# tobwei/APTAI

Measured on AMD Instinct MI355X. Metric: utterances/sec (10 s @ 16 kHz) train-step, higher is better.
Workload: dtype bf16

## Files before the change

### aptai_amd/csrc/attention.hip

```cpp
#include "common.h"

namespace {

#ifdef APTAI_STAMPS
__device__ unsigned long long g_attn_stamps[3 * 1024 * 8];
#define ATTN_STAMP(k, slot)                                                                                       \
    do {                                                                                                          \
        if (threadIdx.x == 0) {                                                                                   \
            const int bl = blockIdx.x + gridDim.x * (blockIdx.y + gridDim.y * blockIdx.z);                        \
            if (bl < 1024) g_attn_stamps[((k) * 1024 + bl) * 8 + (slot)] = wall_clock64();                         \
        }                                                                                                         \
    } while (0)
#else
#define ATTN_STAMP(k, slot) do {} while (0)
#endif

constexpr int HD = 64;
constexpr float LOG2E = 1.4426950408889634f;

struct AttnArgs {
    const bf16_t* qkv; long ld;
    const int* lens;
    bf16_t* ctx; long ldo;
    float* lse2;
// ... 144 lines not shown
    const long tile_stride = 64 * a.ld;
#pragma unroll
    for (int it = 0; it < 2; ++it) { kreg[it] = *(const u32x4*)(Kg + goff[it]); vreg[it] = *(const u32x4*)(Vg + goff[it]); }
    uint32_t hbase = 0;
    if (DROP) hbase = rng_hash((uint32_t)((b * a.heads + hd) * a.Tp + q), a.seed0, a.seed1) + (uint32_t)(2 * h) * ATTN_K1;
    const float c = a.c;
#pragma unroll
    for (int it = 0; it < 2; ++it) { *(u32x4*)(smem + soff[it]) = kreg[it]; *(u32x4*)(smem + 64 * 128 + soff[it]) = vreg[it]; }
    if (ntiles > 1) {
#pragma unroll
        for (int it = 0; it < 2; ++it) {
            kreg[it] = *(const u32x4*)(Kg + tile_stride + goff[it]);
            vreg[it] = *(const u32x4*)(Vg + tile_stride + goff[it]);
        }
    }
    __syncthreads();
    ATTN_STAMP(0, 1);

    auto tile = [&](auto first_flag, auto mask_flag, const int t) {
        constexpr bool FIRST = decltype(first_flag)::value, MASK = decltype(mask_flag)::value;
        const char* sK = smem + (t & 1) * FWD_BUF;
        const char* sV = sK + 64 * 128;
        const int kbase = t * 64;
        bf16x8 kfr[2][4];
#pragma unroll
        for (int ds = 0; ds < 4; ++ds) kfr[0][ds] = rd_row(sK, lo, 0, ds);
        if (t + 1 < ntiles) {
            char* nb = smem + ((t + 1) & 1) * FWD_BUF;
#pragma unroll
            for (int it = 0; it < 2; ++it) { *(u32x4*)(nb + soff[it]) = kreg[it]; *(u32x4*)(nb + 64 * 128 + soff[it]) = vreg[it]; }
            if (t + 2 < ntiles) {
                const bf16_t* kn = Kg + (long)(t + 2) * tile_stride;
                const bf16_t* vn = Vg + (long)(t + 2) * tile_stride;
#pragma unroll
                for (int it = 0; it < 2; ++it) { kreg[it] = *(const u32x4*)(kn + goff[it]); vreg[it] = *(const u32x4*)(vn + goff[it]); }
            }
        }
        f32x16 sT[2];
        sT[0] = __builtin_amdgcn_mfma_f32_32x32x16_bf16(kfr[0][0], qf[0], (f32x16)(0.f), 0, 0, 0);
#pragma unroll
        for (int ds = 1; ds < 4; ++ds) sT[0] = __builtin_amdgcn_mfma_f32_32x32x16_bf16(kfr[0][ds], qf[ds], sT[0], 0, 0, 0);
#pragma unroll
        for (int ds = 0; ds < 4; ++ds) kfr[1][ds] = rd_row(sK, lo, 1, ds);
        sT[1] = __builtin_amdgcn_mfma_f32_32x32x16_bf16(kfr[1][0], qf[0], (f32x16)(0.f), 0, 0, 0);
#pragma unroll
        for (int ds = 1; ds < 4; ++ds) sT[1] = __builtin_amdgcn_mfma_f32_32x32x16_bf16(kfr[1][ds], qf[ds], sT[1], 0, 0, 0);
        if (MASK) {
#pragma unroll
            for (int kt2 = 0; kt2 < 2; ++kt2)
#pragma unroll
                for (int r = 0; r < 16; ++r)
                    if (kbase + kt2 * 32 + acc_row(r, h) >= len) sT[kt2][r] = -INFINITY;
        }
        if (FIRST) {
            float mt = sT[0][0];
#pragma unroll
            for (int r = 1; r < 16; ++r) mt = fmaxf(mt, sT[0][r]);
#pragma unroll
            for (int r = 0; r < 16; ++r) mt = fmaxf(mt, sT[1][r]);
            mt = fmaxf(mt, __shfl_xor(mt, 32, 64));
            ref = fmaf(mt, c, REF_HEADROOM);
        }
        float psum = 0.f;
#pragma unroll
        for (int kt2 = 0; kt2 < 2; ++kt2) {
            bf16x8 vfr[2][2];
#pragma unroll
            for (int s = 0; s < 2; ++s)
#pragma unroll
                for (int dt = 0; dt < 2; ++dt) vfr[s][dt] = rd_tr(sV, lo, 2 * kt2 + s, dt);
            float x[16];
#pragma unroll
            for (int r = 0; r < 16; ++r) { x[r] = fast_exp2(fmaf(sT[kt2][r], c, -ref)); psum += x[r]; }
            if (DROP) {
#pragma unroll
                for (int r = 0; r < 16; r += 2) {
                    const uint32_t hsh = attn_mix(hbase + (uint32_t)(kbase / 2 + 16 * kt2 + acc_row(r, 0) / 2) * ATTN_K1);
                    x[r] = (hsh & 0xffffu) >= a.thr16 ? x[r] : 0.f;
                    x[r + 1] = (hsh >> 16) >= a.thr16 ? x[r + 1] : 0.f;
                }
            }
            const bf16x8 pf0 = pack8(&x[0]), pf1 = pack8(&x[8]);
#pragma unroll
            for (int dt = 0; dt < 2; ++dt) oT[dt] = __builtin_amdgcn_mfma_f32_32x32x16_bf16(vfr[0][dt], pf0, oT[dt], 0, 0, 0);
#pragma unroll
            for (int dt = 0; dt < 2; ++dt) oT[dt] = __builtin_amdgcn_mfma_f32_32x32x16_bf16(vfr[1][dt], pf1, oT[dt], 0, 0, 0);
        }
        psum += __shfl_xor(psum, 32, 64);
        l_run += psum;
        if (!FIRST && __builtin_amdgcn_ballot_w64(!(psum <= REF_SUM_LIMIT))) {
            if (!(psum <= REF_SUM_LIMIT)) {
                const float e = floorf(fast_log2(psum)) + REF_HEADROOM;
                const float sc = fast_exp2(-e);
                ref += e;
                l_run *= sc;
#pragma unroll
                for (int r = 0; r < 16; ++r) { oT[0][r] *= sc; oT[1][r] *= sc; }
            }
        }
        __syncthreads();
    };
    if (ntiles == 1) {
        tile(Flag<true>{}, Flag<true>{}, 0);
    } else {
        tile(Flag<true>{}, Flag<false>{}, 0);
        for (int t = 1; t + 1 < ntiles; ++t) tile(Flag<false>{}, Flag<false>{}, t);
        tile(Flag<false>{}, Flag<true>{}, ntiles - 1);
    }
    ATTN_STAMP(0, 2);
    const float l_tot = l_run;
    const float inv = __frcp_rn(l_tot) * a.dscale;
    if (a.lse2 && h == 0) a.lse2[((long)b * a.heads + hd) * a.Tp + q] = ref + fast_log2(l_tot);
    char* sw = smem + wave * (32 * OUT_PITCH);
    const int r31 = lane & 31;
#pragma unroll
    for (int dt = 0; dt < 2; ++dt)
#pragma unroll
        for (int g4 = 0; g4 < 4; ++g4) {
            oT[dt][4 * g4 + 0] *= inv; oT[dt][4 * g4 + 1] *= inv; oT[dt][4 * g4 + 2] *= inv; oT[dt][4 * g4 + 3] *= inv;
            const int d = dt * 32 + 8 * g4 + 4 * h;
            *(u32x2*)(sw + r31 * OUT_PITCH + d * 2) = (u32x2){pack2bf(oT[dt][4 * g4], oT[dt][4 * g4 + 1]),
                                                              pack2bf(oT[dt][4 * g4 + 2], oT[dt][4 * g4 + 3])};
        }
    __syncthreads();
    const long orow = (rowbase + q0) * a.ldo + hd * HD;
#pragma unroll
    for (int i = 0; i < 4; ++i) {
        const int idx = i * 64 + lane, r = idx >> 3, ch = idx & 7;
        *(u32x4*)(a.ctx + orow + (long)r * a.ldo + ch * 8) = *(const u32x4*)(sw + r * OUT_PITCH + ch * 16);
    }
    if (a.o32) {
#pragma unroll
        for (int dt = 0; dt < 2; ++dt) {
            __syncthreads();
#pragma unroll
            for (int g4 = 0; g4 < 4; ++g4)
                *(f32x4*)(sw + r31 * OUT_PITCH + (8 * g4 + 4 * h) * 4) =
                    (f32x4){oT[dt][4 * g4], oT[dt][4 * g4 + 1], oT[dt][4 * g4 + 2], oT[dt][4 * g4 + 3]};
            __syncthreads();
#pragma unroll
            for (int i = 0; i < 4; ++i) {
                const int idx = i * 64 + lane, r = idx >> 3, ch = idx & 7;
                *(f32x4*)(a.o32 + orow + (long)r * a.ldo + dt * 32 + ch * 4) = *(const f32x4*)(sw + r * OUT_PITCH + ch * 16);
            }
        }
    }
    ATTN_STAMP(0, 3);
#ifdef APTAI_STAMPS
    asm volatile("s_waitcnt vmcnt(0)" ::: "memory");
    ATTN_STAMP(0, 4);
#endif
}

template <bool PRE>
__global__ __launch_bounds__(256, PRE ? DKDV_BLOCKS : 2) void attn_bwd_dkdv_kernel(AttnArgs a) {
    __shared__ __attribute__((aligned(16))) char smem[STAGE_BYTES + 384 + DKDV_KV_BYTES];
    char* sQ = smem;
    char* sD = smem + 32 * 128;
    float* sL = (float*)(smem + STAGE_BYTES);
    char* sKall = smem + STAGE_BYTES + 384;
    char* sVall = sKall + 128 * 128;
    ATTN_STAMP(1, 0);
    if (a.thr16) apply_salt(a.salt, a.seed0, a.seed1);
    const int tid = threadIdx.x, lane = tid & 63, wave = tid >> 6, h = lane >> 5;
    int tile_x, hd, b;
    attn_block(a, tile_x, hd, b);
    const int kb0 = tile_x * 128;
    const int key0 = kb0 + wave * 32;
    int len = a.lens[b];
    len = len < 1 ? 1 : (len > a.Tp ? a.Tp : len);
    const long rowbase = (long)b * a.Tp;
    const int key = key0 + (lane & 31);
    bf16_t* dK0 = a.dqkv + (rowbase + kb0) * a.ld + a.H + hd * HD;
    bf16_t* dV0 = dK0 + a.H;
    if (kb0 >= len) {
        const u32x4 z = {0u, 0u, 0u, 0u};
#pragma unroll
        for (int it = 0; it < 4; ++it) {
            const int cid = it * 256 + tid, row = cid >> 3, ch = cid & 7;
            *(u32x4*)(dK0 + (long)row * a.ld + ch * 8) = z;
            *(u32x4*)(dV0 + (long)row * a.ld + ch * 8) = z;
        }
        return;
    }
    const LaneOffs lo = lane_offs(lane);
    const bf16_t* K0 = a.qkv + (rowbase + kb0) * a.ld + a.H + hd * HD;
    stage_rows128(sKall, K0, a.ld, tid);
    stage_rows128(sVall, K0 + a.H, a.ld, tid);
    f32x16 dKT[2], dVT[2];
    dKT[0] = dKT[1] = dVT[0] = dVT[1] = (f32x16)(0.f);

    const int nq = a.skip_pad_q ? ((len + 31) >> 5) : (a.Tp >> 5);
    const bf16_t* Qb = a.qkv + rowbase * a.ld + hd * HD;
    const bf16_t* Db = a.dctx + rowbase * a.ldo + hd * HD;
    const float* lse = a.lse2 + ((long)b * a.heads + hd) * a.Tp;
    const float* del = a.delta + ((long)b * a.heads + hd) * a.Tp;
    const int srow = tid >> 3, sch = tid & 7;
    const int soff = tile_off(srow, sch);
    const long gq = (long)srow * a.ld + sch * 8, gd = (long)srow * a.ldo + sch * 8;
    u32x4 qreg = *(const u32x4*)(Qb + gq), dreg = *(const u32x4*)(Db + gd);
    const float* stat = (tid < 8 ? lse : del) + (tid & 7) * 4;
    f32x4 sreg = (f32x4)(0.f);
    if (tid < 16) sreg = *(const f32x4*)stat;
    const bool key_ok = key < len;
    const bool wave_boundary = key0 + 32 > len;
    const uint32_t hshift = (key & 1) ? 16u : 0u;
    const float c = a.c;
    const uint32_t pairk = (uint32_t)(key >> 1) * ATTN_K1;
    const uint32_t rowid0 = (uint32_t)((b * a.heads + hd) * a.Tp) + (uint32_t)(tid & 31);
    uint32_t hreg = 0;
    if (a.thr16 && tid >= 32 && tid < 64) hreg = rng_hash(rowid0, a.seed0, a.seed1);
    ATTN_STAMP(1, 1);
    for (int t = 0; t < nq; ++t) {
        __syncthreads();
        *(u32x4*)(sQ + soff) = qreg;
        *(u32x4*)(sD + soff) = dreg;
        if (tid < 16) *(f32x4*)(sL + tid * 4) = PRE ? -sreg : sreg;
        if (a.thr16 && tid >= 32 && tid < 64) ((uint32_t*)sL)[64 + (tid & 31)] = hreg;
        __syncthreads();
        if (t + 1 < nq) {
            qreg = *(const u32x4*)(Qb + (long)(t + 1) * 32 * a.ld + gq);
            dreg = *(const u32x4*)(Db + (long)(t + 1) * 32 * a.ldo + gd);
            if (tid < 16) sreg = *(const f32x4*)(stat + (t + 1) * 32);
            if (a.thr16 && tid >= 32 && tid < 64) hreg = rng_hash(rowid0 + (uint32_t)((t + 1) * 32), a.seed0, a.seed1);
        }
        f32x16 cs = (f32x16)(0.f), cd = (f32x16)(0.f);
        if (PRE) {
#pragma unroll
            for (int g4 = 0; g4 < 4; ++g4) {
                const f32x4 l4 = *(const f32x4*)(sL + 8 * g4 + 4 * h);
                const f32x4 d4 = *(const f32x4*)(sL + 32 + 8 * g4 + 4 * h);
#pragma unroll
                for (int rr = 0; rr < 4; ++rr) { cs[4 * g4 + rr] = l4[rr]; cd[4 * g4 + rr] = d4[rr]; }
            }
        }
        f32x16 s = __builtin_amdgcn_mfma_f32_32x32x16_bf16(rd_row(sQ, lo, 0, 0), rd_row(sKall, lo, wave, 0), cs, 0, 0, 0);
        f32x16 dp = __builtin_amdgcn_mfma_f32_32x32x16_bf16(rd_row(sD, lo, 0, 0), rd_row(sVall, lo, wave, 0), cd, 0, 0, 0);
#pragma unroll
        for (int ds = 1; ds < 4; ++ds) {
            s = __builtin_amdgcn_mfma_f32_32x32x16_bf16(rd_row(sQ, lo, 0, ds), rd_row(sKall, lo, wave, ds), s, 0, 0, 0);
            dp = __builtin_amdgcn_mfma_f32_32x32x16_bf16(rd_row(sD, lo, 0, ds), rd_row(sVall, lo, wave, ds), dp, 0, 0, 0);
        }
        float pd[16], dsv[16];
        if (PRE) {
#pragma unroll
            for (int r = 0; r < 16; ++r) pd[r] = fast_exp2(s[r]);
        } else {
#pragma unroll
            for (int g4 = 0; g4 < 4; ++g4) {
                const f32x4 l4 = *(const f32x4*)(sL + 8 * g4 + 4 * h);
                const f32x4 d4 = *(const f32x4*)(sL + 32 + 8 * g4 + 4 * h);
#pragma unroll
                for (int rr = 0; rr < 4; ++rr) {
                    pd[4 * g4 + rr] = fast_exp2(fmaf(s[4 * g4 + rr], c, -l4[rr]));
                    dsv[4 * g4 + rr] = d4[rr];
                }
            }
        }
        if (wave_boundary) {
#pragma unroll
            for (int r = 0; r < 16; ++r) pd[r] = key_ok ? pd[r] : 0.f;
        }
        if (a.thr16) {
#pragma unroll
            for (int g4 = 0; g4 < 4; ++g4) {
                const u32x4 rh = *(const u32x4*)((const uint32_t*)sL + 64 + 8 * g4 + 4 * h);
                f32x4 nd4 = (f32x4)(0.f);
                if (PRE) nd4 = *(const f32x4*)(sL + 32 + 8 * g4 + 4 * h);
#pragma unroll
                for (int rr = 0; rr < 4; ++rr) {
                    const int r = 4 * g4 + rr;
                    const uint32_t y = attn_mix(rh[rr] + pairk);
                    const bool k = ((y >> hshift) & 0xffffu) >= a.thr16;
                    const float p0 = pd[r];
                    if (PRE) dsv[r] = p0 * (k ? dp[r] : nd4[rr]);
                    else dsv[r] = p0 * ((k ? dp[r] : 0.f) - dsv[r]);
                    pd[r] = k ? p0 : 0.f;
                }
            }
        } else {
#pragma unroll
            for (int r = 0; r < 16; ++r) dsv[r] = PRE ? pd[r] * dp[r] : pd[r] * (dp[r] - dsv[r]);
        }
#pragma unroll
        for (int sstep = 0; sstep < 2; ++sstep) {
            const bf16x8 pf = pack8(&pd[8 * sstep]);
            const bf16x8 df = pack8(&dsv[8 * sstep]);
#pragma unroll
            for (int dt = 0; dt < 2; ++dt) {
                dVT[dt] = __builtin_amdgcn_mfma_f32_32x32x16_bf16(rd_tr(sD, lo, sstep, dt), pf, dVT[dt], 0, 0, 0);
                dKT[dt] = __builtin_amdgcn_mfma_f32_32x32x16_bf16(rd_tr(sQ, lo, sstep, dt), df, dKT[dt], 0, 0, 0);
            }
        }
    }
    __syncthreads();
    ATTN_STAMP(1, 2);
    char* sw = smem + wave * (32 * OUT_PITCH);
    store_rows_bf16(sw, dKT, (PRE ? 0.6931471805599453f : a.scale) * a.dscale, dK0 + (long)(wave * 32) * a.ld, a.ld, lane);
    store_rows_bf16(sw, dVT, a.dscale, dV0 + (long)(wave * 32) * a.ld, a.ld, lane);
    ATTN_STAMP(1, 3);
#ifdef APTAI_STAMPS
    asm volatile("s_waitcnt vmcnt(0)" ::: "memory");
    ATTN_STAMP(1, 4);
#endif
}

template <bool PRE>
__global__ __launch_bounds__(256, 3) void attn_bwd_dq_kernel(AttnArgs a) {
    __shared__ __attribute__((aligned(16))) char smem[DQ_STAGE + 512];
    char* sK = smem;
    char* sV = smem + 32 * 128;
    float* sDel = (float*)(smem + DQ_STAGE);
    ATTN_STAMP(2, 0);
    if (a.thr16) apply_salt(a.salt, a.seed0, a.seed1);
    const int tid = threadIdx.x, lane = tid & 63, wave = tid >> 6, h = lane >> 5;
    int tile_x, hd, b;
    attn_block(a, tile_x, hd, b);
    const int qb0 = tile_x * 128;
    const int q = qb0 + wave * 32 + (lane & 31);
    int len = a.lens[b];
    len = len < 1 ? 1 : (len > a.Tp ? a.Tp : len);
    const long rowbase = (long)b * a.Tp;
    const LaneOffs lo = lane_offs(lane);
    bf16x8 qf[4], df[4];
    const bf16_t* Kb = a.qkv + rowbase * a.ld + a.H + hd * HD;
    const bf16_t* Vb = Kb + a.H;
    const int srow = tid >> 3, sch = tid & 7;
    const int soff = tile_off(srow, sch);
    const long gk = (long)srow * a.ld + sch * 8;
    u32x4 kreg = *(const u32x4*)(Kb + gk), vreg = *(const u32x4*)(Vb + gk);
    const bf16_t* Qrows = a.qkv + (rowbase + qb0) * a.ld + hd * HD;
    const bf16_t* Drows = a.dctx + (rowbase + qb0) * a.ldo + hd * HD;
    u32x4 qst[4], dst[4];
#pragma unroll
    for (int it = 0; it < 4; ++it) {
        const int cid = it * 256 + tid, row = cid >> 3, ch = cid & 7;
        qst[it] = *(const u32x4*)(Qrows + (long)row * a.ld + ch * 8);
        dst[it] = *(const u32x4*)(Drows + (long)row * a.ldo + ch * 8);
    }
    const int part = lane & 15, rsub = lane >> 4;
    f32x4 ovv[8];
#pragma unroll
    for (int it = 0; it < 8; ++it) {
        const int row = wave * 32 + it * 4 + rsub;
        const long g = (rowbase + qb0 + row) * a.ldo + hd * HD + part * 4;
        if (a.o32) {
            ovv[it] = *(const f32x4*)(a.o32 + g);
        } else {
            const u32x2 ov = *(const u32x2*)(a.ctx + g);
            ovv[it] = (f32x4){lo_bf(ov[0]), hi_bf(ov[0]), lo_bf(ov[1]), hi_bf(ov[1])};
        }
    }
    const float lse_q = a.lse2[((long)b * a.heads + hd) * a.Tp + q];
    char* sQt = smem;
    char* sDt = smem + 128 * 128;
#pragma unroll
    for (int it = 0; it < 4; ++it) {
        const int cid = it * 256 + tid, row = cid >> 3, ch = cid & 7;
        *(u32x4*)(sQt + tile_off(row, ch)) = qst[it];
        *(u32x4*)(sDt + tile_off(row, ch)) = dst[it];
    }
    ATTN_STAMP(2, 5);
    __syncthreads();
    ATTN_STAMP(2, 6);
#pragma unroll
    for (int ds = 0; ds < 4; ++ds) { qf[ds] = rd_row(sQt, lo, wave, ds); df[ds] = rd_row(sDt, lo, wave, ds); }
#pragma unroll
    for (int it = 0; it < 8; ++it) {
        const int row = wave * 32 + it * 4 + rsub;
        const u32x2 dv = *(const u32x2*)(sDt + tile_off(row, part >> 1) + ((part & 1) << 3));
        float acc = lo_bf(dv[0]) * ovv[it][0];
        acc = fmaf(hi_bf(dv[0]), ovv[it][1], acc);
        acc = fmaf(lo_bf(dv[1]), ovv[it][2], acc);
        acc = fmaf(hi_bf(dv[1]), ovv[it][3], acc);
        acc += __shfl_xor(acc, 8, 64);
        acc += __shfl_xor(acc, 4, 64);
        acc += __shfl_xor(acc, 2, 64);
        acc += __shfl_xor(acc, 1, 64);
        if (part == 0) sDel[row] = acc;
    }
    ATTN_STAMP(2, 7);
    __syncthreads();
    float del_q = sDel[wave * 32 + (lane & 31)];
    __syncthreads();
    del_q *= __frcp_rn(a.dscale);
    if (h == 0) a.delta[((long)b * a.heads + hd) * a.Tp + q] = del_q;
    f32x16 dQT[2];
    dQT[0] = dQT[1] = (f32x16)(0.f);
    const int nk = (len + 31) >> 5;
    uint32_t hbase = 0;
    if (a.thr16) hbase = rng_hash((uint32_t)((b * a.heads + hd) * a.Tp + q), a.seed0, a.seed1) + (uint32_t)(2 * h) * ATTN_K1;
    const float c = a.c;
    const f32x16 cs = (f32x16)(PRE ? -lse_q : 0.f), cd = (f32x16)(PRE ? -del_q : 0.f);
    ATTN_STAMP(2, 1);
    for (int t = 0; t < nk; ++t) {
        __syncthreads();
        *(u32x4*)(sK + soff) = kreg;
        *(u32x4*)(sV + soff) = vreg;
        __syncthreads();
        if (t + 1 < nk) {
            kreg = *(const u32x4*)(Kb + (long)(t + 1) * 32 * a.ld + gk);
            vreg = *(const u32x4*)(Vb + (long)(t + 1) * 32 * a.ld + gk);
        }
        f32x16 sT = __builtin_amdgcn_mfma_f32_32x32x16_bf16(rd_row(sK, lo, 0, 0), qf[0], cs, 0, 0, 0);
        f32x16 dpT = __builtin_amdgcn_mfma_f32_32x32x16_bf16(rd_row(sV, lo, 0, 0), df[0], cd, 0, 0, 0);
#pragma unroll
        for (int ds = 1; ds < 4; ++ds) {
            sT = __builtin_amdgcn_mfma_f32_32x32x16_bf16(rd_row(sK, lo, 0, ds), qf[ds], sT, 0, 0, 0);
            dpT = __builtin_amdgcn_mfma_f32_32x32x16_bf16(rd_row(sV, lo, 0, ds), df[ds], dpT, 0, 0, 0);
        }
        float dsv[16];
        const bool boundary = t * 32 + 32 > len;
#pragma unroll
        for (int r = 0; r < 16; ++r) {
            float p = PRE ? fast_exp2(sT[r]) : fast_exp2(fmaf(sT[r], c, -lse_q));
            if (boundary && (t * 32 + acc_row(r, h) >= len)) p = 0.f;
            dsv[r] = p;
        }
        if (a.thr16) {
            const float dropped = PRE ? -del_q : 0.f;
#pragma unroll
            for (int r = 0; r < 16; r += 2) {
                const uint32_t hsh = attn_mix(hbase + (uint32_t)(t * 16 + acc_row(r, 0) / 2) * ATTN_K1);
                dpT[r] = (hsh & 0xffffu) >= a.thr16 ? dpT[r] : dropped;
                dpT[r + 1] = (hsh >> 16) >= a.thr16 ? dpT[r + 1] : dropped;
            }
        }
#pragma unroll
        for (int r = 0; r < 16; ++r) dsv[r] *= PRE ? dpT[r] : (dpT[r] - del_q);
#pragma unroll
        for (int sstep = 0; sstep < 2; ++sstep) {
            const bf16x8 dsf = pack8(&dsv[8 * sstep]);
#pragma unroll
            for (int dt = 0; dt < 2; ++dt)
                dQT[dt] = __builtin_amdgcn_mfma_f32_32x32x16_bf16(rd_tr(sK, lo, sstep, dt), dsf, dQT[dt], 0, 0, 0);
        }
    }
    __syncthreads();
    ATTN_STAMP(2, 2);
    store_rows_bf16(smem + wave * (32 * OUT_PITCH), dQT, a.scale * a.dscale,
                    a.dqkv + (rowbase + qb0 + wave * 32) * a.ld + hd * HD, a.ld, lane);
    ATTN_STAMP(2, 3);
#ifdef APTAI_STAMPS
    asm volatile("s_waitcnt vmcnt(0)" ::: "memory");
    ATTN_STAMP(2, 4);
#endif
// ... 475 lines not shown
            for (int it = 0; it < 4; ++it) {
                const int cid = it * 256 + tid, row = cid >> 3, ch = cid & 7;
                *(u32x4*)(dK0 + (long)row * a.ld + ch * 8) = z;
            }
        }
        return;
    }
    const LaneOffs lo = lane_offs(lane);
    const bf16_t* Kg = a.qkv + (rowbase + key) * a.ld + a.H + hd * HD;
    bf16x8 kf[4];
#pragma unroll
    for (int ds = 0; ds < 4; ++ds) kf[ds] = *(const bf16x8*)(Kg + ds * 16 + h * 8);
    f32x16 dKT[2];
    dKT[0] = dKT[1] = (f32x16)(0.f);
    const int nq = a.Tp >> 5;
    const bf16_t* Qb = a.qkv + rowbase * a.ld + hd * HD;
    const float* lse = a.lse2 + bh * a.Tp;
    const float* rsum = pa.rowsum + bh * a.Tp;
    const int srow = tid >> 3, sch = tid & 7;
    const int soff = tile_off(srow, sch);
    const long gq = (long)srow * a.ld + sch * 8;
    u32x4 qreg = *(const u32x4*)(Qb + gq);
    const float* stat = (tid < 8 ? lse : rsum) + (tid & 7) * 4;
    f32x4 sreg = (f32x4)(0.f);
    if (tid < 16) sreg = *(const f32x4*)stat;
    const bool key_ok = key < len;
    const uint32_t hshift = (key & 1) ? 16u : 0u;
    const uint32_t pairk = (uint32_t)(key >> 1) * ATTN_K1;
    const uint32_t rowid0 = (uint32_t)(bh * a.Tp) + (uint32_t)(tid & 31);
    uint32_t hreg = 0;
    if (DROP && tid >= 32 && tid < 64) hreg = rng_hash(rowid0, a.seed0, a.seed1);
    const float c = a.c;
    const float* dPk = pa.dprobs + bh * a.Tp * a.Tp;
    const long tp = a.Tp;
    const uint32_t loff = (uint32_t)(4 * h * a.Tp + key);
    float dreg[16];
#pragma unroll
    for (int r = 0; r < 16; ++r) dreg[r] = (dPk + acc_row(r, 0) * tp)[loff];
#pragma unroll 1
    for (int t = 0; t < nq; ++t) {
        __syncthreads();
        *(u32x4*)(sQ + soff) = qreg;
        if (tid < 16) *(f32x4*)(sL + tid * 4) = sreg;
        if (DROP && tid >= 32 && tid < 64) ((uint32_t*)sL)[64 + (tid & 31)] = hreg;
        __syncthreads();
        if (t + 1 < nq) {
            qreg = *(const u32x4*)(Qb + (long)(t + 1) * 32 * a.ld + gq);
            if (tid < 16) sreg = *(const f32x4*)(stat + (t + 1) * 32);
            if (DROP && tid >= 32 && tid < 64) hreg = rng_hash(rowid0 + (uint32_t)((t + 1) * 32), a.seed0, a.seed1);
        }
        f32x16 s = __builtin_amdgcn_mfma_f32_32x32x16_bf16(rd_row(sQ, lo, 0, 0), kf[0], (f32x16)(0.f), 0, 0, 0);
#pragma unroll
        for (int ds = 1; ds < 4; ++ds) s = __builtin_amdgcn_mfma_f32_32x32x16_bf16(rd_row(sQ, lo, 0, ds), kf[ds], s, 0, 0, 0);
        float dsv[16];
#pragma unroll
        for (int g4 = 0; g4 < 4; ++g4) {
            const f32x4 l4 = *(const f32x4*)(sL + 8 * g4 + 4 * h);
            const f32x4 r4 = *(const f32x4*)(sL + 32 + 8 * g4 + 4 * h);
            u32x4 rh = {0u, 0u, 0u, 0u};
            if (DROP) rh = *(const u32x4*)((const uint32_t*)sL + 64 + 8 * g4 + 4 * h);
#pragma unroll
            for (int rr = 0; rr < 4; ++rr) {
                const int r = 4 * g4 + rr;
                const float p = fast_exp2(fmaf(s[r], c, -l4[rr]));
                float d = dreg[r];
                if (DROP) {
                    const uint32_t y = attn_mix(rh[rr] + pairk);
                    d = ((y >> hshift) & 0xffffu) >= a.thr16 ? d : 0.f;
                }
                dsv[r] = key_ok ? p * (d - r4[rr]) : 0.f;
            }
        }
        __builtin_amdgcn_sched_barrier(0);
        if (t + 1 < nq) {
            const float* dn = dPk + (long)(t + 1) * 32 * tp;
#pragma unroll
            for (int r = 0; r < 16; ++r) dreg[r] = (dn + acc_row(r, 0) * tp)[loff];
        }
#pragma unroll
        for (int sstep = 0; sstep < 2; ++sstep) {
            const bf16x8 df = pack8(&dsv[8 * sstep]);
#pragma unroll
            for (int dt = 0; dt < 2; ++dt)
                dKT[dt] = __builtin_amdgcn_mfma_f32_32x32x16_bf16(rd_tr(sQ, lo, sstep, dt), df, dKT[dt], 0, 0, 0);
        }
    }
    __syncthreads();
    store_rows_bf16_acc(smem + wave * (32 * OUT_PITCH), dKT, (a.q_prescaled ? 0.6931471805599453f : a.scale) * a.dscale,
                        dK0 + (long)(wave * 32) * a.ld, a.ld, lane, pa.accumulate);
}

int fill_args(AttnArgs& a, const char* who, const void* qkv, const int32_t* lens, int64_t B, int64_t Tp, int64_t H,
              int64_t heads, float scale, float dropout_p, uint64_t seed, int q_prescaled, const void* stream) {
    APTAI_REQUIRE(qkv && lens, "%s: null pointer", who);
    APTAI_REQUIRE(B > 0 && Tp > 0 && Tp % 128 == 0, "%s: frames per utterance (%ld) must be a positive multiple of 128", who, (long)Tp);
    APTAI_REQUIRE(heads > 0 && H == heads * HD, "%s: head_dim must be 64 (H=%ld heads=%ld)", who, (long)H, (long)heads);
    memset(&a, 0, sizeof(a));
    a.qkv = (const bf16_t*)qkv; a.ld = 3 * H; a.lens = lens; a.ldo = H;
    a.B = (int)B; a.Tp = (int)Tp; a.H = (int)H; a.heads = (int)heads;
    a.scale = scale; a.c = q_prescaled ? 1.0f : scale * LOG2E;
    a.q_prescaled = q_prescaled;
    a.thr16 = drop_thr16(dropout_p); a.dscale = drop_scale(a.thr16);
    a.seed0 = (uint32_t)seed; a.seed1 = (uint32_t)(seed >> 32);
    a.salt = aptai_seed_salt(stream);
    static const int stagger = getenv("APTAI_ATTN_STAGGER") ? atoi(getenv("APTAI_ATTN_STAGGER")) : 0;
    a.stagger = stagger;
    static const int remap = getenv("APTAI_ATTN_XCD_REMAP") ? atoi(getenv("APTAI_ATTN_XCD_REMAP")) : 1;
    a.xcd_remap = remap;
    return APTAI_OK;
}

}

#ifdef APTAI_STAMPS
extern "C" int aptai_debug_read_attn_stamps(void* host_out) {
    return hipMemcpyFromSymbol(host_out, HIP_SYMBOL(g_attn_stamps), sizeof(g_attn_stamps)) == hipSuccess ? 0 : 1;
}
#endif

extern "C" int aptai_attention_fwd(const void* qkv, const int32_t* lens, void* ctx, float* lse2, float* ctx_f32, int64_t B,
                                   int64_t Tp, int64_t H, int64_t heads, float scale, float dropout_p, uint64_t seed,
                                   int q_prescaled, void* stream_) {
    AttnArgs a;
    int rc = fill_args(a, "aptai_attention_fwd", qkv, lens, B, Tp, H, heads, scale, dropout_p, seed, q_prescaled, stream_);
    if (rc) return rc;
    APTAI_REQUIRE(ctx != nullptr, "aptai_attention_fwd: null ctx");
    a.ctx = (bf16_t*)ctx; a.lse2 = lse2; a.o32 = ctx_f32;
    if (a.thr16) {
        APTAI_LAUNCH(attn_fwd_kernel<true>, dim3((unsigned)(Tp / 128), (unsigned)heads, (unsigned)B), dim3(256), 0,
                     (hipStream_t)stream_, a);
    } else {
        APTAI_LAUNCH(attn_fwd_kernel<false>, dim3((unsigned)(Tp / 128), (unsigned)heads, (unsigned)B), dim3(256), 0,
                     (hipStream_t)stream_, a);
    }
    APTAI_CHECK_LAUNCH("attn_fwd_kernel");
    return APTAI_OK;
}

extern "C" int aptai_attention_bwd(const void* qkv, const int32_t* lens, const void* ctx, const float* ctx_f32, const void* dctx,
                                   const float* lse2, float* delta_ws, void* dqkv, int64_t B, int64_t Tp, int64_t H,
                                   int64_t heads, float scale, float dropout_p, uint64_t seed, int dctx_zero_beyond_len,
                                   int q_prescaled, void* stream_) {
    hipStream_t stream = (hipStream_t)stream_;
    AttnArgs a;
    int rc = fill_args(a, "aptai_attention_bwd", qkv, lens, B, Tp, H, heads, scale, dropout_p, seed, q_prescaled, stream_);
    if (rc) return rc;
    APTAI_REQUIRE(ctx && dctx && lse2 && delta_ws && dqkv, "aptai_attention_bwd: null pointer");
    a.ctx = (bf16_t*)ctx; a.dctx = (const bf16_t*)dctx; a.lse2 = (float*)lse2; a.delta = delta_ws; a.o32 = (float*)ctx_f32; a.dqkv = (bf16_t*)dqkv;
    a.skip_pad_q = dctx_zero_beyond_len;
    dim3 grid((unsigned)(Tp / 128), (unsigned)heads, (unsigned)B);
    if (q_prescaled) {
        APTAI_LAUNCH(attn_bwd_dq_kernel<true>, grid, dim3(256), 0, stream, a);
        APTAI_CHECK_LAUNCH("attn_bwd_dq_kernel");
        APTAI_LAUNCH(attn_bwd_dkdv_kernel<true>, grid, dim3(256), 0, stream, a);
    } else {
        APTAI_LAUNCH(attn_bwd_dq_kernel<false>, grid, dim3(256), 0, stream, a);
        APTAI_CHECK_LAUNCH("attn_bwd_dq_kernel");
        APTAI_LAUNCH(attn_bwd_dkdv_kernel<false>, grid, dim3(256), 0, stream, a);
    }
    APTAI_CHECK_LAUNCH("attn_bwd_dkdv_kernel");
    return APTAI_OK;
}

extern "C" int aptai_attention_probs_fwd(const void* qkv, const int32_t* lens, const float* lse2, float* probs, int64_t B, int64_t Tp,
                                         int64_t H, int64_t heads, float scale, float dropout_p, uint64_t seed, int q_prescaled,
                                         void* stream_) {
    ProbsArgs pa;
    memset(&pa, 0, sizeof(pa));
    int rc = fill_args(pa.a, "aptai_attention_probs_fwd", qkv, lens, B, Tp, H, heads, scale, dropout_p, seed, q_prescaled, stream_);
    if (rc) return rc;
    APTAI_REQUIRE(lse2 && probs, "aptai_attention_probs_fwd: null pointer");
    APTAI_REQUIRE((uintptr_t)probs % 16 == 0, "aptai_attention_probs_fwd: probs must be 16-byte aligned");
    APTAI_REQUIRE(B * heads * Tp < (1L << 31), "aptai_attention_probs_fwd: B * heads * Tp (%ld) exceeds the 32-bit dropout row index",
                  (long)(B * heads * Tp));
    pa.a.lse2 = (float*)lse2; pa.probs = probs;
    const dim3 grid((unsigned)(Tp / 128), (unsigned)heads, (unsigned)B);
    if (pa.a.thr16) {
        APTAI_LAUNCH(attn_probs_fwd_kernel<true>, grid, dim3(256), 0, (hipStream_t)stream_, pa);
    } else {
        APTAI_LAUNCH(attn_probs_fwd_kernel<false>, grid, dim3(256), 0, (hipStream_t)stream_, pa);
    }
    APTAI_CHECK_LAUNCH("attn_probs_fwd_kernel");
    return APTAI_OK;
}

extern "C" int aptai_attention_probs_bwd(const void* qkv, const int32_t* lens, const float* lse2, const float* dprobs, float* rowsum_ws,
                                         void* dqkv, int64_t B, int64_t Tp, int64_t H, int64_t heads, float scale, float dropout_p,
                                         uint64_t seed, int q_prescaled, int accumulate, void* stream_) {
    hipStream_t stream = (hipStream_t)stream_;
    ProbsArgs pa;
    memset(&pa, 0, sizeof(pa));
    int rc = fill_args(pa.a, "aptai_attention_probs_bwd", qkv, lens, B, Tp, H, heads, scale, dropout_p, seed, q_prescaled, stream_);
    if (rc) return rc;
    APTAI_REQUIRE(lse2 && dprobs && rowsum_ws && dqkv, "aptai_attention_probs_bwd: null pointer");
    APTAI_REQUIRE((uintptr_t)dprobs % 16 == 0, "aptai_attention_probs_bwd: dprobs must be 16-byte aligned");
    pa.a.lse2 = (float*)lse2; pa.a.dqkv = (bf16_t*)dqkv; pa.dprobs = dprobs; pa.rowsum = rowsum_ws; pa.accumulate = accumulate;
    const dim3 grid((unsigned)(Tp / 128), (unsigned)heads, (unsigned)B);
    if (pa.a.thr16) {
        APTAI_LAUNCH(attn_probs_bwd_dq_kernel<true>, grid, dim3(256), 0, stream, pa);
        APTAI_CHECK_LAUNCH("attn_probs_bwd_dq_kernel");
        APTAI_LAUNCH(attn_probs_bwd_dk_kernel<true>, grid, dim3(256), 0, stream, pa);
    } else {
        APTAI_LAUNCH(attn_probs_bwd_dq_kernel<false>, grid, dim3(256), 0, stream, pa);
        APTAI_CHECK_LAUNCH("attn_probs_bwd_dq_kernel");
        APTAI_LAUNCH(attn_probs_bwd_dk_kernel<false>, grid, dim3(256), 0, stream, pa);
    }
    APTAI_CHECK_LAUNCH("attn_probs_bwd_dk_kernel");
    return APTAI_OK;
}

extern "C" int aptai_attention_exact_fwd(const void* qkv_split, int64_t ld, const int32_t* lens, void* ctx_split, int64_t ldo, int64_t B,
                                         int64_t Tp, int64_t H, int64_t heads, int pieces, float scale, void* stream_) {
    APTAI_REQUIRE(qkv_split && lens && ctx_split, "aptai_attention_exact_fwd: null pointer");
    APTAI_REQUIRE(B > 0 && Tp > 0 && Tp % 128 == 0, "aptai_attention_exact_fwd: frames per utterance (%ld) must be a positive multiple of 128", (long)Tp);
    APTAI_REQUIRE(heads > 0 && H == heads * HD, "aptai_attention_exact_fwd: head_dim must be 64 (H=%ld heads=%ld)", (long)H, (long)heads);
    APTAI_REQUIRE(pieces == 3 || pieces == 6, "aptai_attention_exact_fwd: pieces must be 3 (f32x3) or 6 (f32x6)");
    APTAI_REQUIRE(ld >= 3 * pieces * H && ld % 8 == 0 && ldo >= pieces * H && ldo % 8 == 0, "aptai_attention_exact_fwd: row pitches (ld=%ld, ldo=%ld) too small "
                  "for %d slots of H=%ld or not a multiple of 8", (long)ld, (long)ldo, pieces, (long)H);
    APTAI_REQUIRE((uintptr_t)qkv_split % 16 == 0 && (uintptr_t)ctx_split % 16 == 0, "aptai_attention_exact_fwd: operands must be 16-byte aligned");
    AttnXArgs a;
    a.qkv = (const bf16_t*)qkv_split; a.ld = ld; a.lens = lens; a.ctx = (bf16_t*)ctx_split; a.ldo = ldo;
    a.B = (int)B; a.Tp = (int)Tp; a.H = (int)H; a.heads = (int)heads; a.slots = pieces;
    a.c = scale * LOG2E;
    static const int remap = getenv("APTAI_ATTN_XCD_REMAP") ? atoi(getenv("APTAI_ATTN_XCD_REMAP")) : 1;
    a.xcd_remap = remap;
    const dim3 grid((unsigned)(Tp / 128), (unsigned)heads, (unsigned)B);
    if (pieces == 3) {
        constexpr int smem = 2 * 2 * 2 * 64 * 128;
        static const hipError_t attr = hipFuncSetAttribute((const void*)attn_exact_fwd_kernel<2>, hipFuncAttributeMaxDynamicSharedMemorySize, smem);
        APTAI_REQUIRE(attr == hipSuccess, "aptai_attention_exact_fwd: cannot reserve %d bytes of LDS", smem);
        APTAI_LAUNCH(attn_exact_fwd_kernel<2>, grid, dim3(256), smem, (hipStream_t)stream_, a);
    } else {
        constexpr int smem = 2 * 2 * 3 * 64 * 128;
        static const hipError_t attr = hipFuncSetAttribute((const void*)attn_exact_fwd_kernel<3>, hipFuncAttributeMaxDynamicSharedMemorySize, smem);
        APTAI_REQUIRE(attr == hipSuccess, "aptai_attention_exact_fwd: cannot reserve %d bytes of LDS", smem);
        APTAI_LAUNCH(attn_exact_fwd_kernel<3>, grid, dim3(256), smem, (hipStream_t)stream_, a);
    }
    APTAI_CHECK_LAUNCH("attn_exact_fwd_kernel");
    return APTAI_OK;
}
```

Before: 1718.

## Hand-schedule dK/dV backward loop: interleave MFMA with LDS reads, exp, dropout masks

Rewrites the inner loop of the attention dK/dV backward kernel as an explicitly software-pipelined sequence. Sched barriers and asm pins interleave each MFMA with the next LDS fragment reads, the exp2 evaluation and the dropout-hash work. Dropout becomes a template parameter so the no-dropout path drops the hash code, and keep masks are stored as wave ballots in scalar registers instead of per-lane bools. The aim is to hide LDS latency and VALU work behind matrix-core issue, at the cost of more register pressure and a rigid, compiler-hostile schedule.

After: 1720 (median of 4 runs). No clear change (+0.1%).

```diff
diff --git a/aptai_amd/csrc/attention.hip b/aptai_amd/csrc/attention.hip
--- a/aptai_amd/csrc/attention.hip
+++ b/aptai_amd/csrc/attention.hip
@@ -320,7 +320,7 @@
 #endif
 }
 
-template <bool PRE>
+template <bool PRE, bool DROP>
 __global__ __launch_bounds__(256, PRE ? DKDV_BLOCKS : 2) void attn_bwd_dkdv_kernel(AttnArgs a) {
     __shared__ __attribute__((aligned(16))) char smem[STAGE_BYTES + 384 + DKDV_KV_BYTES];
     char* sQ = smem;
@@ -329,7 +329,7 @@
     char* sKall = smem + STAGE_BYTES + 384;
     char* sVall = sKall + 128 * 128;
     ATTN_STAMP(1, 0);
-    if (a.thr16) apply_salt(a.salt, a.seed0, a.seed1);
+    if (DROP) apply_salt(a.salt, a.seed0, a.seed1);
     const int tid = threadIdx.x, lane = tid & 63, wave = tid >> 6, h = lane >> 5;
     int tile_x, hd, b;
     attn_block(a, tile_x, hd, b);
@@ -377,89 +377,161 @@
     const uint32_t pairk = (uint32_t)(key >> 1) * ATTN_K1;
     const uint32_t rowid0 = (uint32_t)((b * a.heads + hd) * a.Tp) + (uint32_t)(tid & 31);
     uint32_t hreg = 0;
-    if (a.thr16 && tid >= 32 && tid < 64) hreg = rng_hash(rowid0, a.seed0, a.seed1);
+    if (DROP && tid >= 32 && tid < 64) hreg = rng_hash(rowid0, a.seed0, a.seed1);
     ATTN_STAMP(1, 1);
     for (int t = 0; t < nq; ++t) {
         __syncthreads();
         *(u32x4*)(sQ + soff) = qreg;
         *(u32x4*)(sD + soff) = dreg;
         if (tid < 16) *(f32x4*)(sL + tid * 4) = PRE ? -sreg : sreg;
-        if (a.thr16 && tid >= 32 && tid < 64) ((uint32_t*)sL)[64 + (tid & 31)] = hreg;
+        if (DROP && tid >= 32 && tid < 64) ((uint32_t*)sL)[64 + (tid & 31)] = hreg;
         __syncthreads();
         if (t + 1 < nq) {
             qreg = *(const u32x4*)(Qb + (long)(t + 1) * 32 * a.ld + gq);
             dreg = *(const u32x4*)(Db + (long)(t + 1) * 32 * a.ldo + gd);
             if (tid < 16) sreg = *(const f32x4*)(stat + (t + 1) * 32);
-            if (a.thr16 && tid >= 32 && tid < 64) hreg = rng_hash(rowid0 + (uint32_t)((t + 1) * 32), a.seed0, a.seed1);
-        }
-        f32x16 cs = (f32x16)(0.f), cd = (f32x16)(0.f);
-        if (PRE) {
-#pragma unroll
-            for (int g4 = 0; g4 < 4; ++g4) {
-                const f32x4 l4 = *(const f32x4*)(sL + 8 * g4 + 4 * h);
-                const f32x4 d4 = *(const f32x4*)(sL + 32 + 8 * g4 + 4 * h);
-#pragma unroll
-                for (int rr = 0; rr < 4; ++rr) { cs[4 * g4 + rr] = l4[rr]; cd[4 * g4 + rr] = d4[rr]; }
-            }
-        }
-        f32x16 s = __builtin_amdgcn_mfma_f32_32x32x16_bf16(rd_row(sQ, lo, 0, 0), rd_row(sKall, lo, wave, 0), cs, 0, 0, 0);
-        f32x16 dp = __builtin_amdgcn_mfma_f32_32x32x16_bf16(rd_row(sD, lo, 0, 0), rd_row(sVall, lo, wave, 0), cd, 0, 0, 0);
-#pragma unroll
-        for (int ds = 1; ds < 4; ++ds) {
-            s = __builtin_amdgcn_mfma_f32_32x32x16_bf16(rd_row(sQ, lo, 0, ds), rd_row(sKall, lo, wave, ds), s, 0, 0, 0);
-            dp = __builtin_amdgcn_mfma_f32_32x32x16_bf16(rd_row(sD, lo, 0, ds), rd_row(sVall, lo, wave, ds), dp, 0, 0, 0);
-        }
+            if (DROP && tid >= 32 && tid < 64) hreg = rng_hash(rowid0 + (uint32_t)((t + 1) * 32), a.seed0, a.seed1);
+        }
+        const float* sLl = sL + 4 * h;
+        const float* sLd = sL + 32 + 4 * h;
+        f32x16 s = (f32x16)(0.f), dp = (f32x16)(0.f);
         float pd[16], dsv[16];
-        if (PRE) {
-#pragma unroll
-            for (int r = 0; r < 16; ++r) pd[r] = fast_exp2(s[r]);
-        } else {
-#pragma unroll
-            for (int g4 = 0; g4 < 4; ++g4) {
-                const f32x4 l4 = *(const f32x4*)(sL + 8 * g4 + 4 * h);
-                const f32x4 d4 = *(const f32x4*)(sL + 32 + 8 * g4 + 4 * h);
-#pragma unroll
-                for (int rr = 0; rr < 4; ++rr) {
-                    pd[4 * g4 + rr] = fast_exp2(fmaf(s[4 * g4 + rr], c, -l4[rr]));
-                    dsv[4 * g4 + rr] = d4[rr];
-                }
-            }
-        }
+        uint64_t kp[16];
+        bf16x8 fa[4], fb[4], ga[4], gb[4];
+        u32x4 rh[4];
+#define DKDV_RH(G4) if (DROP) rh[G4] = *(const u32x4*)((const uint32_t*)sL + 64 + 8 * (G4) + 4 * h);
+#define DKDV_PIN(ACC)                                                                                              \
+        asm volatile("" : "+v"(ACC) :: "memory");                                                                 \
+        __builtin_amdgcn_sched_barrier(0);
+#define DKDV_EXP(R0, R1)                                                                                           \
+        _Pragma("unroll") for (int r = (R0); r < (R1); ++r) pd[r] = PRE ? fast_exp2(s[r]) : fast_exp2(fmaf(s[r], c, -dsv[r]));
+#define DKDV_ROWS(DST, BASE)                                                                                       \
+        _Pragma("unroll") for (int g4 = 0; g4 < 4; ++g4) {                                                        \
+            const f32x4 v4 = *(const f32x4*)((BASE) + 8 * g4);                                                    \
+            _Pragma("unroll") for (int rr = 0; rr < 4; ++rr) DST[4 * g4 + rr] = v4[rr];                           \
+        }
+#define DKDV_KEEP(G4)                                                                                              \
+        if (DROP) {                                                                                               \
+            _Pragma("unroll") for (int rr = 0; rr < 4; ++rr) {                                                    \
+                const uint32_t y = attn_mix(rh[G4][rr] + pairk);                                                    \
+                kp[4 * (G4) + rr] = __builtin_amdgcn_ballot_w64(((y >> hshift) & 0xffffu) >= a.thr16);            \
+                asm volatile("" : "+s"(kp[4 * (G4) + rr]));                    \
+            }                                                                                                     \
+        }
+        if (PRE) { DKDV_ROWS(s, sLl) }
+#pragma unroll
+        for (int ds = 0; ds < 2; ++ds) { fa[ds] = rd_row(sQ, lo, 0, ds); fb[ds] = rd_row(sKall, lo, wave, ds); }
+        DKDV_RH(0)
+        __builtin_amdgcn_sched_barrier(0);
+        s = __builtin_amdgcn_mfma_f32_32x32x16_bf16(fa[0], fb[0], s, 0, 0, 0);
+        DKDV_PIN(s);
+        fa[2] = rd_row(sQ, lo, 0, 2); fb[2] = rd_row(sKall, lo, wave, 2);
+        DKDV_RH(1)
+        DKDV_KEEP(0)
+        __builtin_amdgcn_sched_barrier(0);
+        s = __builtin_amdgcn_mfma_f32_32x32x16_bf16(fa[1], fb[1], s, 0, 0, 0);
+        DKDV_PIN(s);
+        fa[3] = rd_row(sQ, lo, 0, 3); fb[3] = rd_row(sKall, lo, wave, 3);
+        DKDV_RH(2)
+        DKDV_KEEP(1)
+        __builtin_amdgcn_sched_barrier(0);
+        s = __builtin_amdgcn_mfma_f32_32x32x16_bf16(fa[2], fb[2], s, 0, 0, 0);
+        DKDV_PIN(s);
+        ga[0] = rd_row(sD, lo, 0, 0); gb[0] = rd_row(sVall, lo, wave, 0);
+        DKDV_RH(3)
+        if (PRE) { DKDV_ROWS(dp, sLd) }
+        DKDV_KEEP(2)
+        __builtin_amdgcn_sched_barrier(0);
+        s = __builtin_amdgcn_mfma_f32_32x32x16_bf16(fa[3], fb[3], s, 0, 0, 0);
+        DKDV_PIN(s);
+        ga[1] = rd_row(sD, lo, 0, 1); gb[1] = rd_row(sVall, lo, wave, 1);
+        if (!PRE) { DKDV_ROWS(dsv, sLl) }
+        DKDV_KEEP(3)
+        __builtin_amdgcn_sched_barrier(0);
+        dp = __builtin_amdgcn_mfma_f32_32x32x16_bf16(ga[0], gb[0], dp, 0, 0, 0);
+        DKDV_PIN(dp);
+        ga[2] = rd_row(sD, lo, 0, 2); gb[2] = rd_row(sVall, lo, wave, 2);
+        DKDV_EXP(0, 4)
+        __builtin_amdgcn_sched_barrier(0);
+        dp = __builtin_amdgcn_mfma_f32_32x32x16_bf16(ga[1], gb[1], dp, 0, 0, 0);
+        DKDV_PIN(dp);
+        ga[3] = rd_row(sD, lo, 0, 3); gb[3] = rd_row(sVall, lo, wave, 3);
+        DKDV_EXP(4, 8)
+        __builtin_amdgcn_sched_barrier(0);
+        dp = __builtin_amdgcn_mfma_f32_32x32x16_bf16(ga[2], gb[2], dp, 0, 0, 0);
+        DKDV_PIN(dp);
+        bf16x8 td[2][2], tq[2][2];
+        td[0][0] = rd_tr(sD, lo, 0, 0); td[0][1] = rd_tr(sD, lo, 0, 1);
+        DKDV_EXP(8, 12)
+        __builtin_amdgcn_sched_barrier(0);
+        dp = __builtin_amdgcn_mfma_f32_32x32x16_bf16(ga[3], gb[3], dp, 0, 0, 0);
+        DKDV_PIN(dp);
+        td[1][0] = rd_tr(sD, lo, 1, 0); td[1][1] = rd_tr(sD, lo, 1, 1);
+        DKDV_EXP(12, 16)
+        if (!PRE) { DKDV_ROWS(dsv, sLd) }
+#undef DKDV_EXP
+#undef DKDV_PIN
+#undef DKDV_ROWS
+#undef DKDV_KEEP
+#undef DKDV_RH
         if (wave_boundary) {
 #pragma unroll
             for (int r = 0; r < 16; ++r) pd[r] = key_ok ? pd[r] : 0.f;
         }
-        if (a.thr16) {
-#pragma unroll
-            for (int g4 = 0; g4 < 4; ++g4) {
-                const u32x4 rh = *(const u32x4*)((const uint32_t*)sL + 64 + 8 * g4 + 4 * h);
+        auto keptp = [&](const int sstep) {
+            float pm[8];
+#pragma unroll
+            for (int j = 0; j < 8; ++j) {
+                const int r = 8 * sstep + j;
+                pm[j] = (DROP && !__builtin_amdgcn_inverse_ballot_w64(kp[r])) ? 0.f : pd[r];
+            }
+            return pack8(pm);
+        };
+        auto ds8 = [&](const int sstep) {
+#pragma unroll
+            for (int g4 = 2 * sstep; g4 < 2 * sstep + 2; ++g4) {
                 f32x4 nd4 = (f32x4)(0.f);
-                if (PRE) nd4 = *(const f32x4*)(sL + 32 + 8 * g4 + 4 * h);
+                if (PRE && DROP) nd4 = *(const f32x4*)(sL + 32 + 8 * g4 + 4 * h);
 #pragma unroll
                 for (int rr = 0; rr < 4; ++rr) {
                     const int r = 4 * g4 + rr;
-                    const uint32_t y = attn_mix(rh[rr] + pairk);
-                    const bool k = ((y >> hshift) & 0xffffu) >= a.thr16;
                     const float p0 = pd[r];
-                    if (PRE) dsv[r] = p0 * (k ? dp[r] : nd4[rr]);
-                    else dsv[r] = p0 * ((k ? dp[r] : 0.f) - dsv[r]);
-                    pd[r] = k ? p0 : 0.f;
+                    if (DROP) {
+                        const bool k = __builtin_amdgcn_inverse_ballot_w64(kp[r]);
+                        if (PRE) dsv[r] = p0 * (k ? dp[r] : nd4[rr]);
+                        else dsv[r] = p0 * ((k ? dp[r] : 0.f) - dsv[r]);
+                    } else {
+                        dsv[r] = PRE ? p0 * dp[r] : p0 * (dp[r] - dsv[r]);
+                    }
                 }
             }
-        } else {
-#pragma unroll
-            for (int r = 0; r < 16; ++r) dsv[r] = PRE ? pd[r] * dp[r] : pd[r] * (dp[r] - dsv[r]);
-        }
-#pragma unroll
-        for (int sstep = 0; sstep < 2; ++sstep) {
-            const bf16x8 pf = pack8(&pd[8 * sstep]);
-            const bf16x8 df = pack8(&dsv[8 * sstep]);
-#pragma unroll
-            for (int dt = 0; dt < 2; ++dt) {
-                dVT[dt] = __builtin_amdgcn_mfma_f32_32x32x16_bf16(rd_tr(sD, lo, sstep, dt), pf, dVT[dt], 0, 0, 0);
-                dKT[dt] = __builtin_amdgcn_mfma_f32_32x32x16_bf16(rd_tr(sQ, lo, sstep, dt), df, dKT[dt], 0, 0, 0);
-            }
-        }
+            return pack8(&dsv[8 * sstep]);
+        };
+#define DKDV_PIN(ACC)                                                                                              \
+        asm volatile("" : "+v"(ACC) :: "memory");                                                                 \
+        __builtin_amdgcn_sched_barrier(0);
+        const bf16x8 pf0 = keptp(0);
+        __builtin_amdgcn_sched_barrier(0);
+        dVT[0] = __builtin_amdgcn_mfma_f32_32x32x16_bf16(td[0][0], pf0, dVT[0], 0, 0, 0);
+        dVT[1] = __builtin_amdgcn_mfma_f32_32x32x16_bf16(td[0][1], pf0, dVT[1], 0, 0, 0);
+        DKDV_PIN(dVT[1]);
+        const bf16x8 pf1 = keptp(1);
+        __builtin_amdgcn_sched_barrier(0);
+        dVT[0] = __builtin_amdgcn_mfma_f32_32x32x16_bf16(td[1][0], pf1, dVT[0], 0, 0, 0);
+        dVT[1] = __builtin_amdgcn_mfma_f32_32x32x16_bf16(td[1][1], pf1, dVT[1], 0, 0, 0);
+        DKDV_PIN(dVT[1]);
+        tq[0][0] = rd_tr(sQ, lo, 0, 0); tq[0][1] = rd_tr(sQ, lo, 0, 1);
+        const bf16x8 df0 = ds8(0);
+        tq[1][0] = rd_tr(sQ, lo, 1, 0); tq[1][1] = rd_tr(sQ, lo, 1, 1);
+        __builtin_amdgcn_sched_barrier(0);
+        dKT[0] = __builtin_amdgcn_mfma_f32_32x32x16_bf16(tq[0][0], df0, dKT[0], 0, 0, 0);
+        dKT[1] = __builtin_amdgcn_mfma_f32_32x32x16_bf16(tq[0][1], df0, dKT[1], 0, 0, 0);
+        DKDV_PIN(dKT[1]);
+        const bf16x8 df1 = ds8(1);
+        __builtin_amdgcn_sched_barrier(0);
+        dKT[0] = __builtin_amdgcn_mfma_f32_32x32x16_bf16(tq[1][0], df1, dKT[0], 0, 0, 0);
+        dKT[1] = __builtin_amdgcn_mfma_f32_32x32x16_bf16(tq[1][1], df1, dKT[1], 0, 0, 0);
+#undef DKDV_PIN
     }
     __syncthreads();
     ATTN_STAMP(1, 2);
@@ -1241,11 +1313,13 @@
     if (q_prescaled) {
         APTAI_LAUNCH(attn_bwd_dq_kernel<true>, grid, dim3(256), 0, stream, a);
         APTAI_CHECK_LAUNCH("attn_bwd_dq_kernel");
-        APTAI_LAUNCH(attn_bwd_dkdv_kernel<true>, grid, dim3(256), 0, stream, a);
+        if (a.thr16) APTAI_LAUNCH((attn_bwd_dkdv_kernel<true, true>), grid, dim3(256), 0, stream, a);
+        else APTAI_LAUNCH((attn_bwd_dkdv_kernel<true, false>), grid, dim3(256), 0, stream, a);
     } else {
         APTAI_LAUNCH(attn_bwd_dq_kernel<false>, grid, dim3(256), 0, stream, a);
         APTAI_CHECK_LAUNCH("attn_bwd_dq_kernel");
-        APTAI_LAUNCH(attn_bwd_dkdv_kernel<false>, grid, dim3(256), 0, stream, a);
+        if (a.thr16) APTAI_LAUNCH((attn_bwd_dkdv_kernel<false, true>), grid, dim3(256), 0, stream, a);
+        else APTAI_LAUNCH((attn_bwd_dkdv_kernel<false, false>), grid, dim3(256), 0, stream, a);
     }
     APTAI_CHECK_LAUNCH("attn_bwd_dkdv_kernel");
     return APTAI_OK;
```
